# FREDZEL2020/jittor-MYC-NeRFs

Measured on AMD Instinct MI355X. Metric: ray_samples_per_sec, higher is better.
Workload: dtype f32 (emulated: 3 x f16-split MFMA products, fp32 accumulate; fp32 VALU elsewhere); 1 GPU; TensorVMSplit 300^3 (16/48 comps, MLP_Fea 150-128-128-3), 800x800 rays x 512 samples/ray (BASELINE configs[1]); ONE frame per step at every N (N>1: split over the ranks, BASELINE configs[2]), 512-ray tiles round-robin, one RCCL all_gather of [4 cap] fp32 (rgb block + depth block, written in place by the render) + two strided un-permute copies; scene=synthetic scene A (SURVEY 8d), no alpha mask, white_bg, samples_per_ray=512, rays_per_rank=640000, tile=512, chunk=640000, alpha_mask=0, emulate_world=0, arith=f32

## Files before the change

### jittor-myc-nerfs_amd/csrc/tvr_march.hip

```cpp
#include <cstdlib>
#include "tvr_device.h"
#include "tvr_kernels.h"
#include "tvr_march_body.h"
#include "tvr_gradient.h"


template <bool DENSE, bool LDSL>
__global__ __launch_bounds__(64 * MARCH_MAX_WAVES) void march_kernel(const SceneDev sc, const float *__restrict__ rays,
                                                                     const int n_rays, const int S, const int s_cap,
                                                                     const MarchSampling sm, const float eps_T,
                                                                     MarchOut mo, const tvr_dense_out dn)
{
    constexpr bool CP = false, VOL = false;
    const CpDev cp = {};
    const float *const dvol = nullptr;
#include "tvr_march_body.inc"
}

template <bool DENSE, bool PLAIN, bool BATCH>
__global__ __launch_bounds__(64 * MARCH_VOL_WAVES, DENSE ? MARCH_VOL_OCC - 1 : MARCH_VOL_OCC) void march_vol_kernel(const SceneDev sc, const float *__restrict__ dvol, const float *__restrict__ rays,
                                                                         const int n_rays, const int S, const int s_cap, const MarchSampling sm, const float eps_T,
                                                                         MarchOut mo, const tvr_dense_out dn)
{
    static_assert(!(PLAIN && DENSE), "the plain form has no dense outputs");
    constexpr bool LDSL = false, CP = false, VOL = true, MARCH_BATCH = BATCH;
    const CpDev cp = {};
#include "tvr_march_body.inc"
}

__global__ __launch_bounds__(256) void density_volume_kernel(const SceneDev sc, float *__restrict__ out)
{
    const long long gx1 = sc.grid[0] + 1, gy1 = sc.grid[1] + 1, gz1 = sc.grid[2] + 1;
    const long long t = (long long)blockIdx.x * blockDim.x + threadIdx.x;
    if (t >= gx1 * gy1 * gz1) return;
    const long long x = t % gx1, y = (t / gx1) % gy1, z = t / (gx1 * gy1);
    const float4 *P[3] = {sc.dplane[0] + (y * gx1 + x) * 4, sc.dplane[1] + (z * gx1 + x) * 4, sc.dplane[2] + (z * gy1 + y) * 4};
    const float4 *Ln[3] = {sc.dline[0] + z * 4, sc.dline[1] + y * 4, sc.dline[2] + x * 4};
    double acc = 0.0;
#pragma unroll
    for (int i = 0; i < 3; ++i) {
#pragma unroll
        for (int g = 0; g < 4; ++g) {
            const float4 p = P[i][g], l = Ln[i][g];
            acc = acc + (double)p.x * (double)l.x;
            acc = acc + (double)p.y * (double)l.y;
            acc = acc + (double)p.z * (double)l.z;
            acc = acc + (double)p.w * (double)l.w;
        }
    }
    out[t] = (float)acc;
}

hipError_t launch_density_volume(const SceneDev &sc, float *out, hipStream_t stream)
{
    const long long n = ((long long)sc.grid[0] + 1) * ((long long)sc.grid[1] + 1) * ((long long)sc.grid[2] + 1);
    hipLaunchKernelGGL(density_volume_kernel, dim3((unsigned)((n + 255) / 256)), dim3(256), 0, stream, sc, out);
    return hipGetLastError();
}

#define COMP_LANES 8
__global__ __launch_bounds__(256) void composite_kernel(const MarchOut mo, const int n_rays, const int white_bg,
                                                        float *__restrict__ rgb_out)
{
    const int t = blockIdx.x * blockDim.x + threadIdx.x;
    const int r = t / COMP_LANES, l = t % COMP_LANES;
    const bool live = r < n_rays;
    const unsigned base = live ? mo.ray_off[r] : 0u, cnt = live ? mo.ray_cnt[r] : 0u;
    float c0 = 0.f, c1 = 0.f, c2 = 0.f;
    unsigned i = l;
    for (; i + 3 * COMP_LANES < cnt; i += 4 * COMP_LANES) {
        const float4 e0 = mo.q_out[base + i], e1 = mo.q_out[base + i + COMP_LANES], e2 = mo.q_out[base + i + 2 * COMP_LANES],
                     e3 = mo.q_out[base + i + 3 * COMP_LANES];
        c0 = c0 + e0.w * e0.x; c1 = c1 + e0.w * e0.y; c2 = c2 + e0.w * e0.z;
        c0 = c0 + e1.w * e1.x; c1 = c1 + e1.w * e1.y; c2 = c2 + e1.w * e1.z;
        c0 = c0 + e2.w * e2.x; c1 = c1 + e2.w * e2.y; c2 = c2 + e2.w * e2.z;
        c0 = c0 + e3.w * e3.x; c1 = c1 + e3.w * e3.y; c2 = c2 + e3.w * e3.z;
    }
    for (; i < cnt; i += COMP_LANES) {
        const float4 e = mo.q_out[base + i];
        c0 = c0 + e.w * e.x;
        c1 = c1 + e.w * e.y;
        c2 = c2 + e.w * e.z;
    }
#pragma unroll
    for (int off = 1; off < COMP_LANES; off <<= 1) {
        c0 = c0 + __shfl_xor(c0, off);
        c1 = c1 + __shfl_xor(c1, off);
        c2 = c2 + __shfl_xor(c2, off);
    }
    if (!live || l != 0) return;
    if (mo.counter[2] != 0u) {
        const float qnan = __int_as_float(0x7fc00000);
        rgb_out[(size_t)r * 3 + 0] = qnan; rgb_out[(size_t)r * 3 + 1] = qnan; rgb_out[(size_t)r * 3 + 2] = qnan;
        mo.depth[r] = qnan;
        return;
    }
    const float acc = mo.acc[r];
    if (white_bg) {
        const float bg = 1.0f - acc;
        c0 = c0 + bg; c1 = c1 + bg; c2 = c2 + bg;
    }
    rgb_out[(size_t)r * 3 + 0] = clamp01(c0);
    rgb_out[(size_t)r * 3 + 1] = clamp01(c1);
    rgb_out[(size_t)r * 3 + 2] = clamp01(c2);
}

__global__ __launch_bounds__(256) void scatter_rgb_kernel(const MarchOut mo, const int S, float *__restrict__ rgb_dense)
{
    const unsigned n = *mo.counter;
    for (unsigned e = blockIdx.x * blockDim.x + threadIdx.x; e < n; e += gridDim.x * blockDim.x) {
        const float4 v = mo.q_out[e];
        const size_t q = ((size_t)mo.q_ray[e] * S + mo.q_j[e]) * 3;
        rgb_dense[q] = v.x; rgb_dense[q + 1] = v.y; rgb_dense[q + 2] = v.z;
    }
}

__global__ __launch_bounds__(256) void density_feature_kernel(const SceneDev sc, const float *__restrict__ xyz, const long long m,
                                                              float *__restrict__ out)
{
    const long long t = (long long)blockIdx.x * blockDim.x + threadIdx.x;
    const long long s = t >> 2;
    const int sub = threadIdx.x & 3;
    float part = 0.0f;
    if (s < m) {
        int i0[3];
        float w[3];
#pragma unroll
        for (int k = 0; k < 3; ++k) {
            const float f = unnorm(xyz[s * 3 + k], sc.gm1[k]);
            const float fl = floorf(fminf(fmaxf(f, -2.0f), sc.gm1[k] + 2.0f));
            i0[k] = (int)fl;
            w[k] = f - fl;
        }
        const float4 a = vm_term<4, true>(sc.dplane[0], sc.dline[0], sc.grid[0], sc.grid[1], sc.grid[2], i0[0], i0[1], i0[2], w[0], w[1], w[2], sub);
        const float4 b = vm_term<4, true>(sc.dplane[1], sc.dline[1], sc.grid[0], sc.grid[2], sc.grid[1], i0[0], i0[2], i0[1], w[0], w[2], w[1], sub);
        const float4 c = vm_term<4, true>(sc.dplane[2], sc.dline[2], sc.grid[1], sc.grid[2], sc.grid[0], i0[1], i0[2], i0[0], w[1], w[2], w[0], sub);
        part = ((a.x + a.y) + (a.z + a.w)) + ((b.x + b.y) + (b.z + b.w)) + ((c.x + c.y) + (c.z + c.w));
    }
    part += __shfl_xor(part, 1);
    part += __shfl_xor(part, 2);
    if (s < m && sub == 0) out[s] = part;
}

__global__ __launch_bounds__(256) void density_gradient_kernel(const SceneDev sc, const float *__restrict__ xyz, const long long m, const float3 h, const float3 inv2h,
                                                               float *__restrict__ sigma_feature, float *__restrict__ grad)
{
    const long long t = (long long)blockIdx.x * blockDim.x + threadIdx.x;
    const long long s = t >> 2;
    const int sub = threadIdx.x & 3;
    float f[7];
#pragma unroll
    for (int j = 0; j < 7; ++j) f[j] = 0.0f;
    if (s < m) vm_grad_point(sc, xyz[s * 3], xyz[s * 3 + 1], xyz[s * 3 + 2], h, sub, f);
#pragma unroll
    for (int j = 0; j < 7; ++j) {
        f[j] += __shfl_xor(f[j], 1);
        f[j] += __shfl_xor(f[j], 2);
    }
    if (s < m && sub == 0) {
        if (sigma_feature) sigma_feature[s] = f[0];
        grad[s * 3 + 0] = (f[1] - f[2]) * inv2h.x;
        grad[s * 3 + 1] = (f[3] - f[4]) * inv2h.y;
        grad[s * 3 + 2] = (f[5] - f[6]) * inv2h.z;
    }
}

__global__ __launch_bounds__(256) void alpha_sample_kernel(const SceneDev sc, const float *__restrict__ xyz, const long long m,
                                                           float *__restrict__ out)
{
    const long long s = (long long)blockIdx.x * blockDim.x + threadIdx.x;
    if (s >= m) return;
    const float p[3] = {xyz[s * 3], xyz[s * 3 + 1], xyz[s * 3 + 2]};
    out[s] = alpha_lookup(sc, p);
}

__global__ __launch_bounds__(256) void alpha_bits_kernel(const float *__restrict__ vol, const long long n, unsigned *__restrict__ bits)
{
    const long long wd = (long long)blockIdx.x * blockDim.x + threadIdx.x;
    if (wd * 32 >= n) return;
    unsigned v = 0u;
    for (int b = 0; b < 32; ++b) {
        const long long i = wd * 32 + b;
        if (i < n && vol[i] > 0.0f) v |= 1u << b;
    }
    bits[wd] = v;
}

hipError_t launch_alpha_bits(const float *vol, long long n, unsigned *bits, hipStream_t stream)
{
    const long long words = (n + 31) / 32;
    hipLaunchKernelGGL(alpha_bits_kernel, dim3((unsigned)((words + 255) / 256)), dim3(256), 0, stream, vol, n, bits);
    return hipGetLastError();
}

template <bool DENSE, bool LDSL>
static hipError_t launch_march_t(const SceneDev &sc, const float *rays, int n_rays, int S, const MarchSampling &sm, float eps_T, const MarchOut &mo,
                                 const tvr_dense_out &dn, int waves, size_t lds, unsigned grid, hipStream_t stream)
{
    hipError_t rc = hipFuncSetAttribute((const void *)march_kernel<DENSE, LDSL>, hipFuncAttributeMaxDynamicSharedMemorySize, (int)lds);
    if (rc != hipSuccess) return rc;
    hipLaunchKernelGGL((march_kernel<DENSE, LDSL>), dim3(grid), dim3(64 * waves), lds, stream, sc, rays, n_rays, S, S, sm, eps_T, mo, dn);
    return hipGetLastError();
}

static int device_cu_count()
{
    static int cus = 0;
    if (cus == 0) {
        int dev = 0, n = 0;
        if (hipGetDevice(&dev) == hipSuccess && hipDeviceGetAttribute(&n, hipDeviceAttributeMultiprocessorCount, dev) == hipSuccess && n > 0) cus = n;
        else cus = 256;
    }
    return cus;
}

int march_cu_count() { return device_cu_count(); }

static hipError_t launch_march_vol(const SceneDev &sc, const float *dvol, const float *rays, int n_rays, int S, const MarchSampling &sm, float eps_T, const MarchOut &mo,
                                   const tvr_dense_out *dense, hipStream_t stream)
{
    const int groups = MARCH_VOL_GROUPS;
    const size_t kLds = 160 * 1024 / (size_t)groups, per_list = (size_t)S * 6, fixed = MARCH_HDR + 64;
    const int n_tiles = (n_rays + MARCH_TILE - 1) / MARCH_TILE;
    int waves = 1;
    size_t lds = 0;
    long long grid = 1;
    auto shape = [&](size_t per_pend) {
        const int w = (int)((kLds - fixed - (per_pend ? 16 : 0)) / (per_list + per_pend));
        waves = w >= MARCH_VOL_WAVES ? MARCH_VOL_WAVES : (w >= 8 ? 8 : (w >= 4 ? 4 : (w >= 2 ? 2 : 1)));
        lds = per_pend ? fixed + (((size_t)waves * per_list + 15) & ~(size_t)15) + (size_t)waves * per_pend : fixed + (size_t)waves * per_list;
        grid = (long long)device_cu_count() * groups * (MARCH_VOL_WAVES / waves);
        if (grid > n_tiles) grid = n_tiles;
        if (grid < 1) grid = 1;
    };
    shape(0);
    const bool batch = (long long)n_rays > grid * (long long)waves;
    if (batch) shape((size_t)MARCH_PEND * MARCH_PEND_WORDS * 4);
    tvr_dense_out none = {};
    const tvr_dense_out &dn = dense ? *dense : none;
    const unsigned long long vol_bytes = 4ull * (unsigned long long)(sc.grid[0] + 1) * (unsigned long long)(sc.grid[1] + 1) * (unsigned long long)(sc.grid[2] + 1);
    const bool plain = !dense && sc.avol == nullptr && sm.zv == nullptr && mo.lam6 == nullptr && vol_bytes < (1ull << 32);
    hipError_t rc = hipSuccess;
    auto go = [&](auto kern) {
        rc = hipFuncSetAttribute((const void *)kern, hipFuncAttributeMaxDynamicSharedMemorySize, (int)lds);
        if (rc == hipSuccess) hipLaunchKernelGGL(kern, dim3((unsigned)grid), dim3(64 * waves), lds, stream, sc, dvol, rays, n_rays, S, S, sm, eps_T, mo, dn);
    };
    if (dense) batch ? go(march_vol_kernel<true, false, true>) : go(march_vol_kernel<true, false, false>);
    else if (plain) batch ? go(march_vol_kernel<false, true, true>) : go(march_vol_kernel<false, true, false>);
    else batch ? go(march_vol_kernel<false, false, true>) : go(march_vol_kernel<false, false, false>);
    if (rc != hipSuccess) return rc;
    return hipGetLastError();
}

hipError_t launch_march(const SceneDev &sc, const float *rays, int n_rays, int S, const MarchSampling &sm, float eps_T,
                        const MarchOut &mo, const tvr_dense_out *dense, hipStream_t stream, const float *dvol)
{
    if (dvol) return launch_march_vol(sc, dvol, rays, n_rays, S, sm, eps_T, mo, dense, stream);
    const size_t kLds = 160 * 1024, line_bytes = ((size_t)sc.grid[0] + sc.grid[1] + sc.grid[2] + 3) * 16 * MARCH_LSTRIDE, per_wave = (size_t)S * 6;
    bool ldsl = MARCH_HDR + line_bytes + 4 * per_wave + 64 <= kLds;
    const size_t fixed = MARCH_HDR + (ldsl ? line_bytes : 0) + 64;
    int waves = (int)((kLds - fixed) / per_wave);
    waves = waves >= 16 ? 16 : (waves >= 12 ? 12 : (waves >= 8 ? 8 : (waves >= 4 ? 4 : (waves >= 2 ? 2 : 1))));
    const size_t lds = fixed + (size_t)waves * per_wave;
    const int n_tiles = (n_rays + MARCH_TILE - 1) / MARCH_TILE;
    long long grid = (long long)device_cu_count() * (16 / waves > 0 ? 16 / waves : 1);
    if (grid > n_tiles) grid = n_tiles;
    if (grid < 1) grid = 1;
    tvr_dense_out none = {};
    const tvr_dense_out &dn = dense ? *dense : none;
    if (dense) return ldsl ? launch_march_t<true, true>(sc, rays, n_rays, S, sm, eps_T, mo, dn, waves, lds, (unsigned)grid, stream)
                           : launch_march_t<true, false>(sc, rays, n_rays, S, sm, eps_T, mo, dn, waves, lds, (unsigned)grid, stream);
    return ldsl ? launch_march_t<false, true>(sc, rays, n_rays, S, sm, eps_T, mo, dn, waves, lds, (unsigned)grid, stream)
                : launch_march_t<false, false>(sc, rays, n_rays, S, sm, eps_T, mo, dn, waves, lds, (unsigned)grid, stream);
}

hipError_t launch_composite(const MarchOut &mo, int n_rays, int white_bg, float *rgb, hipStream_t stream)
{
    const long long threads = (long long)n_rays * COMP_LANES;
    hipLaunchKernelGGL(composite_kernel, dim3((unsigned)((threads + 255) / 256)), dim3(256), 0, stream, mo, n_rays, white_bg, rgb);
    return hipGetLastError();
}

hipError_t launch_scatter_rgb(const MarchOut &mo, int S, float *rgb_dense, hipStream_t stream)
{
    hipLaunchKernelGGL(scatter_rgb_kernel, dim3(1024), dim3(256), 0, stream, mo, S, rgb_dense);
    return hipGetLastError();
}

hipError_t launch_density_feature(const SceneDev &sc, const float *xyz, long long m, float *out, hipStream_t stream)
{
    const long long blocks = (m * 4 + 255) / 256;
    hipLaunchKernelGGL(density_feature_kernel, dim3((unsigned)blocks), dim3(256), 0, stream, sc, xyz, m, out);
    return hipGetLastError();
}

hipError_t launch_density_gradient(const SceneDev &sc, const float *xyz, long long m, const float h[3], const float inv2h[3], float *sigma_feature, float *grad,
                                   hipStream_t stream)
{
    const long long blocks = (m * 4 + 255) / 256;
    hipLaunchKernelGGL(density_gradient_kernel, dim3((unsigned)blocks), dim3(256), 0, stream, sc, xyz, m, make_float3(h[0], h[1], h[2]),
                       make_float3(inv2h[0], inv2h[1], inv2h[2]), sigma_feature, grad);
    return hipGetLastError();
}

hipError_t launch_alpha_sample(const SceneDev &sc, const float *xyz, long long m, float *out, hipStream_t stream)
{
    hipLaunchKernelGGL(alpha_sample_kernel, dim3((unsigned)((m + 255) / 256)), dim3(256), 0, stream, sc, xyz, m, out);
    return hipGetLastError();
}
```

### jittor-myc-nerfs_amd/csrc/tvr_march_body.h

```cpp
#pragma once
#include "tvr_device.h"
#include "tvr_kernels.h"

#define MARCH_MAX_WAVES 16
#define MARCH_TILE 16
#define MARCH_SPIN_LIMIT (1u << 22)
#define MARCH_SLOTS 64u
#ifndef MARCH_CTR_WORD
#define MARCH_CTR_WORD 1
#endif
#ifndef MARCH_TAIL
#define MARCH_TAIL 4u
#endif
#ifndef MARCH_VOL_WAVES
#define MARCH_VOL_WAVES 16
#endif
#ifndef MARCH_VOL_GROUPS
#define MARCH_VOL_GROUPS 1
#endif
#ifndef MARCH_VOL_OCC
#define MARCH_VOL_OCC 8
#endif
#define MARCH_HDR 560
#ifndef MARCH_LSTRIDE
#define MARCH_LSTRIDE 4
#endif

__device__ __forceinline__ float4 vm_term_lds(const float4 *__restrict__ P, const float4 *Ls, int W, int x0, int y0, int l0,
                                              float wx, float wy, float wl, int sub)
{
    const float ux = 1.0f - wx, uy = 1.0f - wy, ul = 1.0f - wl;
    const int Wp = W + 1;
    const unsigned cell = __umul24((unsigned)y0, (unsigned)Wp) + (unsigned)x0;
    unsigned o0 = (cell << 6) + ((unsigned)sub << 4), o1 = o0 + ((unsigned)Wp << 6);
    asm volatile("" : "+v"(o0), "+v"(o1));
    const unsigned char *pb = (const unsigned char *)P;
    const float4 t00 = *(const float4 *)(pb + (size_t)o0), t01 = *(const float4 *)(pb + (size_t)o0 + 64);
    const float4 t10 = *(const float4 *)(pb + (size_t)o1), t11 = *(const float4 *)(pb + (size_t)o1 + 64);
    const float4 *q = Ls + l0 * MARCH_LSTRIDE + sub;
    const float4 l0v = q[0], l1v = q[MARCH_LSTRIDE];
    float4 p4 = f4_mul(ux * uy, t00);
    p4 = f4_fma(wx * uy, t01, p4);
    p4 = f4_fma(ux * wy, t10, p4);
    p4 = f4_fma(wx * wy, t11, p4);
    float4 q4 = f4_mul(ul, l0v);
    q4 = f4_fma(wl, l1v, q4);
    return make_float4(p4.x * q4.x, p4.y * q4.y, p4.z * q4.z, p4.w * q4.w);
}

__device__ __forceinline__ float cp_density_quad(const SceneDev &sc, const CpDev &cp, int ix, int iy, int iz, float wx, float wy, float wz, int sub)
{
    const int tpt = cp.rd >> 2;
    const float4 *__restrict__ l0 = sc.dline[0] + (size_t)iz * tpt + sub;
    const float4 *__restrict__ l1 = sc.dline[1] + (size_t)iy * tpt + sub;
    const float4 *__restrict__ l2 = sc.dline[2] + (size_t)ix * tpt + sub;
    const float ux = 1.0f - wx, uy = 1.0f - wy, uz = 1.0f - wz;
    float part = 0.0f;
    for (int g = 0; g < tpt; g += 4) {
        const float4 a0 = l0[g], a1 = l0[g + tpt], b0 = l1[g], b1 = l1[g + tpt], c0 = l2[g], c1 = l2[g + tpt];
        const float4 a = f4_fma(wz, a1, f4_mul(uz, a0)), b = f4_fma(wy, b1, f4_mul(uy, b0)), c = f4_fma(wx, c1, f4_mul(ux, c0));
        const float tx = (a.x * b.x) * c.x, ty = (a.y * b.y) * c.y, tz = (a.z * b.z) * c.z, tw = (a.w * b.w) * c.w;
        part = part + ((tx + ty) + (tz + tw));
    }
    return part;
}

struct __attribute__((packed, aligned(4))) vol_pair { float a, b; };
__device__ __forceinline__ float vol_density(const float *__restrict__ D, int gx1, int gy1, int ix, int iy, int iz, float wx, float wy, float wz)
{
    const size_t sy = (size_t)gx1, sz = (size_t)gx1 * (size_t)gy1;
    const float *r = D + ((size_t)iz * sz + (size_t)iy * sy + (size_t)ix);
    const vol_pair p00 = *(const vol_pair *)r, p01 = *(const vol_pair *)(r + sy);
    const vol_pair p10 = *(const vol_pair *)(r + sz), p11 = *(const vol_pair *)(r + sz + sy);
    const float c00 = __builtin_fmaf(wx, p00.b - p00.a, p00.a), c01 = __builtin_fmaf(wx, p01.b - p01.a, p01.a);
    const float c10 = __builtin_fmaf(wx, p10.b - p10.a, p10.a), c11 = __builtin_fmaf(wx, p11.b - p11.a, p11.a);
    const float c0 = __builtin_fmaf(wy, c01 - c00, c00), c1 = __builtin_fmaf(wy, c11 - c10, c10);
    return __builtin_fmaf(wz, c1 - c0, c0);
}

constexpr bool PLAIN = false;

constexpr bool MARCH_BATCH = false;
#define MARCH_PEND 8
#define MARCH_PEND_WORDS 12

struct MarchVolArgs {
    SceneDev sc;
    const float *dvol, *rays;
    int n_rays, S, s_cap;
    MarchSampling sm;
    float eps_T;
    MarchOut mo;
    tvr_dense_out dn;
};
template <bool ON_DEMAND, typename T>
__device__ __forceinline__ T march_arg_now(const T &arg, unsigned offset)
{
#if defined(__HIP_DEVICE_COMPILE__)
    if constexpr (ON_DEMAND) {
        const __attribute__((address_space(4))) unsigned char *ka = (const __attribute__((address_space(4))) unsigned char *)__builtin_amdgcn_kernarg_segment_ptr();
        asm volatile("" : "+s"(ka));
        return *(const __attribute__((address_space(4))) T *)(ka + offset);
    }
#endif
    return arg;
}

__device__ __forceinline__ float vol_density32(const unsigned char *r00, const unsigned char *r01, const unsigned char *r10, const unsigned char *r11, unsigned gx1,
                                               unsigned gy1, int ix, int iy, int iz, float wx, float wy, float wz)
{
    const unsigned row = __umul24((unsigned)iz, gy1) + (unsigned)iy;
    unsigned o = (row * gx1 + (unsigned)ix) << 2;
    asm volatile("" : "+v"(o));
    const vol_pair p00 = *(const vol_pair *)(r00 + (size_t)o), p01 = *(const vol_pair *)(r01 + (size_t)o);
    const vol_pair p10 = *(const vol_pair *)(r10 + (size_t)o), p11 = *(const vol_pair *)(r11 + (size_t)o);
    const float c00 = __builtin_fmaf(wx, p00.b - p00.a, p00.a), c01 = __builtin_fmaf(wx, p01.b - p01.a, p01.a);
    const float c10 = __builtin_fmaf(wx, p10.b - p10.a, p10.a), c11 = __builtin_fmaf(wx, p11.b - p11.a, p11.a);
    const float c0 = __builtin_fmaf(wy, c01 - c00, c00), c1 = __builtin_fmaf(wy, c11 - c10, c10);
    return __builtin_fmaf(wz, c1 - c0, c0);
}

#ifndef MARCH_VOL_LEAN
#define MARCH_VOL_LEAN 1
#endif
__device__ __forceinline__ float march_expf(float x)
{
    const float p = x * 0x1.715476p+0f;
    const float r = __builtin_rintf(p);
    float lo = __builtin_fmaf(x, 0x1.715476p+0f, -p);
    lo = __builtin_fmaf(x, 0x1.4ae0bep-26f, lo);
    return __builtin_ldexpf(__builtin_amdgcn_exp2f((p - r) + lo), (int)r);
}
__device__ __forceinline__ float march_softplus(float x)
{
    if (x > 20.0f) return x;
    const float t = march_expf(x);
    const float u = 1.0f + t, d = u - 1.0f;
    const float rc = __builtin_amdgcn_rcpf(d);
    float q = t * rc;
    q = __builtin_fmaf(__builtin_fmaf(-d, q, t), rc, q);
    const float lg = __builtin_amdgcn_logf(u) * 0x1.62e430p-1f;
    return d == 0.0f ? t : lg * q;
}

#define MARCH_DPP_WAVE_SHR1 0x138
#define MARCH_DPP_SAME 0xE4
template <int CTRL, int ROWS>
__device__ __forceinline__ float march_dpp_mov(float old, float v)
{
    return __int_as_float(__builtin_amdgcn_update_dpp(__float_as_int(old), __float_as_int(v), CTRL, ROWS, 0xF, false));
}
template <int N>
__device__ __forceinline__ float march_up(float v)
{
    float t = march_dpp_mov<MARCH_DPP_WAVE_SHR1, 0xF>(1.0f, v);
#pragma unroll
    for (int i = 1; i < N; ++i) t = march_dpp_mov<MARCH_DPP_WAVE_SHR1, 0xF>(t, t);
    return t;
}
__device__ __forceinline__ void scan_mul_dpp(float &x, float &excl, float &last)
{
    x = x * march_up<1>(x);
    x = x * march_up<2>(x);
    x = x * march_up<4>(x);
    x = x * march_up<8>(x);
    {
        const auto q = __builtin_amdgcn_permlane16_swap(__float_as_uint(x), __float_as_uint(x), false, false);
        const auto s = __builtin_amdgcn_permlane32_swap(q[0], q[1], false, false);
        float t = march_dpp_mov<MARCH_DPP_SAME, 0x6>(1.0f, __uint_as_float(s[0]));
        t = march_dpp_mov<MARCH_DPP_SAME, 0x8>(t, __uint_as_float(q[0]));
        x = x * t;
    }
    {
        const auto h = __builtin_amdgcn_permlane32_swap(__float_as_uint(x), __float_as_uint(x), false, false);
        x = x * march_dpp_mov<MARCH_DPP_SAME, 0xC>(1.0f, __uint_as_float(h[0]));
    }
    excl = march_up<1>(x);
    last = __int_as_float(__builtin_amdgcn_readlane(__float_as_int(x), 63));
}

template <bool PLAIN_F>
__device__ __forceinline__ void march_flush(const SceneDev &sc, const MarchSampling &sm, const MarchOut &mo, const int S, const int s_cap, const int lane, const float *bufw,
                                            const unsigned short *bufj, const float *pend, int &ring_head, int &pend_total, int &n_pend)
{
    __builtin_amdgcn_fence(__ATOMIC_ACQ_REL, "wavefront");
    const MarchOut mf = march_arg_now<PLAIN_F>(mo, offsetof(MarchVolArgs, mo));
    const bool jit_f = march_arg_now<PLAIN_F>(sm.jitter, offsetof(MarchVolArgs, sm.jitter)) != nullptr;
    const int f_total = __builtin_amdgcn_readfirstlane(pend_total), f_rays = __builtin_amdgcn_readfirstlane(n_pend), f_head = __builtin_amdgcn_readfirstlane(ring_head);
    unsigned fbase = 0;
    if (lane == 0) fbase = atomicAdd(mf.counter, (unsigned)f_total);
    fbase = __builtin_amdgcn_readfirstlane(fbase);
    if (lane < f_rays) mf.ray_off[__float_as_uint(pend[lane * MARCH_PEND_WORDS + 8])] = fbase + __float_as_uint(pend[lane * MARCH_PEND_WORDS + 9]);
    for (int i = lane; i < f_total; i += 64) {
        int k = 0;
        for (int m = 1; m < f_rays; ++m) k += (unsigned)i >= __float_as_uint(pend[m * MARCH_PEND_WORDS + 9]) ? 1 : 0;
        const float *rec = pend + k * MARCH_PEND_WORDS;
        int rp = f_head + i;
        if (rp >= s_cap) rp -= s_cap;
        const unsigned ej = bufj[rp];
        const unsigned eray = __float_as_uint(rec[8]);
        float fj = (float)ej;
        if (jit_f) fj = fj + rec[7];
        const float *__restrict__ zr = (!PLAIN_F && sm.zv) ? sm.zv + (size_t)eray * S : nullptr;
        const float z = zr ? zr[ej] : rec[6] + sc.step * fj;
        float4 qv;
        qv.x = ((rec[0] + rec[3] * z) - sc.lo[0]) * sc.inv[0] - 1.0f;
        qv.y = ((rec[1] + rec[4] * z) - sc.lo[1]) * sc.inv[1] - 1.0f;
        qv.z = ((rec[2] + rec[5] * z) - sc.lo[2]) * sc.inv[2] - 1.0f;
        qv.w = bufw[rp];
        mf.q_pos[fbase + i] = qv;
        mf.q_ray[fbase + i] = eray;
        if (mf.q_j) mf.q_j[fbase + i] = ej;
    }
    __builtin_amdgcn_fence(__ATOMIC_ACQ_REL, "wavefront");
    ring_head = f_head + f_total >= s_cap ? f_head + f_total - s_cap : f_head + f_total;
    pend_total = 0;
    n_pend = 0;
    asm volatile("" : "+v"(ring_head), "+v"(pend_total), "+v"(n_pend));
}
```

### jittor-myc-nerfs_amd/csrc/tvr_march_body.inc

```
    static_assert(!(CP && LDSL), "the CP lines (up to 96 channels) do not go through LDS");
    static_assert(!(VOL && (CP || LDSL)), "the baked volume replaces the factored evaluation: no lines in LDS, no CP lines");
    extern __shared__ __attribute__((aligned(16))) unsigned char lds_raw[];
    const int lane = threadIdx.x & 63;
    const int wave = __builtin_amdgcn_readfirstlane(threadIdx.x >> 6);
    const int n_waves = blockDim.x >> 6;
    unsigned *cursor = (unsigned *)lds_raw;
    const float4 *ls0 = (const float4 *)(lds_raw + MARCH_HDR);
    const int ln0 = LDSL ? (sc.grid[2] + 1) * MARCH_LSTRIDE : 0, ln1 = LDSL ? (sc.grid[1] + 1) * MARCH_LSTRIDE : 0, ln2 = LDSL ? (sc.grid[0] + 1) * MARCH_LSTRIDE : 0;
    const float4 *ls1 = ls0 + ln0, *ls2 = ls1 + ln1;
    float *bufw = (float *)(ls2 + ln2) + (size_t)wave * s_cap;
    unsigned short *bufj = (unsigned short *)((float *)(ls2 + ln2) + (size_t)n_waves * s_cap) + (size_t)wave * s_cap;
#ifdef TVR_MARCH_TIMELINE
    unsigned long long tl_chunks = 0ull, tl_rays = 0ull, tl_resv = 0ull;
    if (mo.stats && threadIdx.x == 0) mo.stats[32 + 8 * blockIdx.x] = __builtin_amdgcn_s_memrealtime();
#endif
    if (threadIdx.x == 0) *cursor = 0u;
    unsigned long long *slots = (unsigned long long *)(lds_raw + 16);
    if (threadIdx.x < MARCH_SLOTS) slots[threadIdx.x] = 0ull;
    unsigned long long *gstat = (unsigned long long *)(lds_raw + 16 + 8 * MARCH_SLOTS);
    if (threadIdx.x < 3) gstat[threadIdx.x] = 0ull;
    if (LDSL) {
        float4 *dst = (float4 *)(lds_raw + MARCH_HDR);
        for (int i = threadIdx.x; i < (sc.grid[2] + 1) * 4; i += blockDim.x) dst[(i >> 2) * MARCH_LSTRIDE + (i & 3)] = sc.dline[0][i];
        for (int i = threadIdx.x; i < (sc.grid[1] + 1) * 4; i += blockDim.x) dst[ln0 + (i >> 2) * MARCH_LSTRIDE + (i & 3)] = sc.dline[1][i];
        for (int i = threadIdx.x; i < (sc.grid[0] + 1) * 4; i += blockDim.x) dst[ln0 + ln1 + (i >> 2) * MARCH_LSTRIDE + (i & 3)] = sc.dline[2][i];
    }
    __syncthreads();
#ifdef TVR_MARCH_TIMELINE
    if (mo.stats && threadIdx.x == 0) mo.stats[32 + 8 * blockIdx.x + 1] = __builtin_amdgcn_s_memrealtime();
#endif
    const int sub = lane & 3;
    const unsigned char *vrow[4] = {nullptr, nullptr, nullptr, nullptr};
    if constexpr (PLAIN) {
        const size_t vsy = (size_t)(sc.grid[0] + 1) * 4, vsz = vsy * (size_t)(sc.grid[1] + 1);
        vrow[0] = (const unsigned char *)dvol; vrow[1] = vrow[0] + vsy; vrow[2] = vrow[0] + vsz; vrow[3] = vrow[2] + vsy;
    }
    unsigned long long clk0 = 0ull, ref0 = 0ull;
    if (march_arg_now<PLAIN>(mo.stats, offsetof(MarchVolArgs, mo.stats)) && threadIdx.x == 0) { clk0 = __builtin_amdgcn_s_memtime(); ref0 = __builtin_amdgcn_s_memrealtime(); }

    unsigned long long st_eval = 0, st_bbox = 0, st_term = 0;
    int last_start = 0;

    int ring_head = 0, pend_total = 0, n_pend = 0;
    float *pend = nullptr;
    if constexpr (MARCH_BATCH) {
        pend = (float *)(lds_raw + ((MARCH_HDR + (size_t)n_waves * s_cap * 6 + 15) & ~(size_t)15)) + (size_t)wave * (MARCH_PEND * MARCH_PEND_WORDS);
        asm volatile("" : "+v"(ring_head), "+v"(pend_total), "+v"(n_pend));
    }

    for (;;) {
        unsigned ci = 0;
        if (lane == 0) ci = atomicAdd(cursor, 1u);
        ci = __builtin_amdgcn_readfirstlane(ci);
        int ray_start, ray_len;
        {
            const unsigned k = ci / MARCH_TILE, slot = k & (MARCH_SLOTS - 1u);
            if ((ci % MARCH_TILE) == 0u) {
                unsigned t = 0, len = MARCH_TILE;
                if (lane == 0) {
                    if ((long long)n_rays >= 8LL * MARCH_TILE * (long long)gridDim.x && (long long)last_start + 2LL * MARCH_TILE * (long long)gridDim.x >= (long long)n_rays)
                        len = MARCH_TAIL;
                    t = atomicAdd(march_arg_now<PLAIN>(mo.counter, offsetof(MarchVolArgs, mo.counter)) + MARCH_CTR_WORD, len);
                    const unsigned long long genw = (unsigned long long)(k + 1u) | (len == MARCH_TAIL ? 0x80000000ull : 0ull);
#ifdef TVR_FAULT_INJECT_MARCH
                    if (blockIdx.x == 0 && k == 3u) __hip_atomic_store(&slots[slot], ((unsigned long long)(k + 1u + MARCH_SLOTS) << 32) | t, __ATOMIC_RELEASE, __HIP_MEMORY_SCOPE_WORKGROUP);
                    else
#endif
                    __hip_atomic_store(&slots[slot], (genw << 32) | t, __ATOMIC_RELEASE, __HIP_MEMORY_SCOPE_WORKGROUP);
                }
                ray_start = (int)__builtin_amdgcn_readfirstlane(t);
                ray_len = (int)__builtin_amdgcn_readfirstlane(len);
            } else {
                unsigned long long v;
                unsigned spins = 0u, fault = 0u;
                for (;;) {
                    v = __hip_atomic_load(&slots[slot], __ATOMIC_ACQUIRE, __HIP_MEMORY_SCOPE_WORKGROUP);
                    const unsigned gen = (unsigned)(v >> 32) & 0x7fffffffu;
                    if (gen == k + 1u) break;
                    if (gen > k + 1u) { fault = 1u; break; }
                    if (++spins > MARCH_SPIN_LIMIT) { fault = 2u; break; }
                    __builtin_amdgcn_s_sleep(1);
                }
                if (fault) {
                    if (lane == 0) atomicOr(march_arg_now<PLAIN>(mo.counter, offsetof(MarchVolArgs, mo.counter)) + 2, fault);
                    break;
                }
                ray_start = (int)(unsigned)v;
                ray_len = (v >> 63) ? MARCH_TAIL : MARCH_TILE;
            }
        }
        if (ray_start >= n_rays) break;
        if ((int)(ci % MARCH_TILE) >= ray_len) continue;
        last_start = ray_start;
        const int ray = ray_start + (int)(ci % MARCH_TILE);
        if (ray >= n_rays) continue;
        const float *__restrict__ const rays_r = march_arg_now<PLAIN>(rays, offsetof(MarchVolArgs, rays));
        const float *const jit_r = march_arg_now<PLAIN>(sm.jitter, offsetof(MarchVolArgs, sm.jitter));
        float o[3], d[3];
#pragma unroll
        for (int k = 0; k < 3; ++k) {
            o[k] = rays_r[(size_t)ray * 6 + k];
            d[k] = rays_r[(size_t)ray * 6 + 3 + k];
        }
        const float tmin = ray_tmin(sc, o, d);
        const bool has_jit = jit_r != nullptr;
        const float u = has_jit ? jit_r[ray] : 0.0f;
        const float *__restrict__ zrow = (!PLAIN && sm.zv) ? sm.zv + (size_t)ray * S : nullptr;
        float lam6 = 1.0f;
        int n6 = 0;

        float T = 1.0f, acc_l = 0.0f, dep_l = 0.0f;
        int napp = 0;
        bool seen = false, terminated = false;
        int c = 0;
        bool make_room = false;
        for (;;) {
        for (; c * 64 < S; ++c) {
            if constexpr (MARCH_BATCH) {
                if (__ballot(n_pend > 0 && (n_pend == MARCH_PEND || pend_total + napp + 64 > s_cap))) { make_room = true; break; }
            }
            const int j = c * 64 + lane;
            const bool inr = j < S;
            float fj = (float)j, fj1 = (float)(j + 1);
            if (has_jit) { fj = fj + u; fj1 = fj1 + u; }
            float z = tmin + sc.step * fj;
            float z1 = tmin + sc.step * fj1;
            if (zrow) {
                z = inr ? zrow[j] : 0.0f;
                z1 = (j < S - 1) ? zrow[j + 1] : z;
            }
            float p[3], n[3], f[3];
            bool bbox = inr;
#pragma unroll
            for (int k = 0; k < 3; ++k) {
                p[k] = o[k] + d[k] * z;
                bbox = bbox & !((sc.lo[k] > p[k]) | (p[k] > sc.hi[k]));
            }
            bool valid = bbox;
            if (!PLAIN && sc.avol != nullptr) {
                if (bbox) valid = sc.abits ? alpha_positive(sc, p) : (alpha_lookup(sc, p) > 0.0f);
            }
            int i0[3];
            float w[3];
#pragma unroll
            for (int k = 0; k < 3; ++k) {
                n[k] = (p[k] - sc.lo[k]) * sc.inv[k] - 1.0f;
                f[k] = unnorm(n[k], sc.gm1[k]);
                const float fl = floorf(f[k]);
                i0[k] = (int)fl;
                w[k] = f[k] - fl;
            }
            if constexpr (PLAIN) asm volatile("" : "+v"(i0[0]), "+v"(i0[1]), "+v"(i0[2]), "+v"(w[0]), "+v"(w[1]), "+v"(w[2]));
            const unsigned long long mb = __ballot(bbox), mv = __ballot(valid);
            if (DENSE) {
                const size_t q = (size_t)ray * S + j;
                if (inr) {
                    if (dn.z) dn.z[q] = z;
                    if (dn.valid) dn.valid[q] = valid;
                    if (dn.bbox_valid) dn.bbox_valid[q] = bbox;
                    if (dn.cell) { dn.cell[q * 3] = i0[0]; dn.cell[q * 3 + 1] = i0[1]; dn.cell[q * 3 + 2] = i0[2]; }
                }
            }
            st_bbox += __popcll(mb);
            if (mv == 0ull) {
                if (DENSE && inr) {
                    const size_t q = (size_t)ray * S + j;
                    if (dn.sigma_feature) dn.sigma_feature[q] = 0.f;
                    if (dn.sigma) dn.sigma[q] = 0.f;
                    if (dn.alpha) dn.alpha[q] = 0.f;
                    if (dn.weight) dn.weight[q] = 0.f;
                }
                if (mb == 0ull && seen && !DENSE) break;
                continue;
            }
            seen = true;
            st_eval += __popcll(mv);
#ifdef TVR_MARCH_TIMELINE
            tl_chunks++;
#endif

            float sf = 0.0f;
            if constexpr (VOL) {
                if constexpr (PLAIN) {
                    if (valid) sf = vol_density32(vrow[0], vrow[1], vrow[2], vrow[3], (unsigned)(sc.grid[0] + 1), (unsigned)(sc.grid[1] + 1), i0[0], i0[1], i0[2], w[0], w[1], w[2]);
                } else
                if (valid) sf = vol_density(dvol, sc.grid[0] + 1, sc.grid[1] + 1, i0[0], i0[1], i0[2], w[0], w[1], w[2]);
            } else {
#pragma unroll
                for (int k4 = 0; k4 < 4; ++k4) {
                    const bool v = quad_bcast_i((int)valid, k4) != 0;
                    if (__ballot(v) == 0ull) continue;
                    const int ix = quad_bcast_i(i0[0], k4), iy = quad_bcast_i(i0[1], k4), iz = quad_bcast_i(i0[2], k4);
                    const float wx = quad_bcast_f(w[0], k4), wy = quad_bcast_f(w[1], k4), wz = quad_bcast_f(w[2], k4);
                    float part = 0.0f;
                    if constexpr (CP) {
                        if (v) part = cp_density_quad(sc, cp, ix, iy, iz, wx, wy, wz, sub);
                    } else
                    if (v && LDSL) {
                        const float4 a = vm_term_lds(sc.dplane[0], ls0, sc.grid[0], ix, iy, iz, wx, wy, wz, sub);
                        const float4 b = vm_term_lds(sc.dplane[1], ls1, sc.grid[0], ix, iz, iy, wx, wz, wy, sub);
                        const float4 cc = vm_term_lds(sc.dplane[2], ls2, sc.grid[1], iy, iz, ix, wy, wz, wx, sub);
                        part = ((a.x + a.y) + (a.z + a.w)) + ((b.x + b.y) + (b.z + b.w)) + ((cc.x + cc.y) + (cc.z + cc.w));
                    } else if (v) {
                        const float4 a = vm_term<4, false>(sc.dplane[0], sc.dline[0], sc.grid[0], sc.grid[1], sc.grid[2], ix, iy, iz, wx, wy, wz, sub);
                        const float4 b = vm_term<4, false>(sc.dplane[1], sc.dline[1], sc.grid[0], sc.grid[2], sc.grid[1], ix, iz, iy, wx, wz, wy, sub);
                        const float4 cc = vm_term<4, false>(sc.dplane[2], sc.dline[2], sc.grid[1], sc.grid[2], sc.grid[0], iy, iz, ix, wy, wz, wx, sub);
                        part = ((a.x + a.y) + (a.z + a.w)) + ((b.x + b.y) + (b.z + b.w)) + ((cc.x + cc.y) + (cc.z + cc.w));
                    }
                    part += quad_perm_f<QUAD_XOR1>(part);
                    part += quad_perm_f<QUAD_XOR2>(part);
                    if (sub == k4) sf = part;
                }
            }

            float sigma = 0.0f;
            constexpr bool LEAN = VOL && MARCH_VOL_LEAN;
            if constexpr (LEAN) {
                if (valid) sigma = (sc.act == 0) ? march_softplus(sf + sc.shift) : fmaxf(sf, 0.0f);
            } else
            if (valid) sigma = (sc.act == 0) ? softplus_f(sf + sc.shift) : fmaxf(sf, 0.0f);
            float dist = (j < S - 1) ? (z1 - z) : 0.0f;
            dist = dist * sc.scale;
            const float alpha = 1.0f - (LEAN ? march_expf(-sigma * dist) : expf(-sigma * dist));
            const float fT = (1.0f - alpha) + 1e-10f;
            if (!PLAIN && mo.lam6) {
                float f6 = inr ? (1.0f - alpha) + 1e-6f : 1.0f;
#pragma unroll
                for (int off = 32; off > 0; off >>= 1) f6 = f6 * __shfl_xor(f6, off);
                lam6 = lam6 * f6;
                n6 += min(64, S - c * 64);
            }
            float incl = fT, excl, last;
            if constexpr (VOL) {
                scan_mul_dpp(incl, excl, last);
            } else {
#pragma unroll
                for (int off = 1; off < 64; off <<= 1) {
                    const float t = __shfl_up(incl, off);
                    if (lane >= off) incl = incl * t;
                }
                excl = __shfl_up(incl, 1);
                if (lane == 0) excl = 1.0f;
            }
            const float Tj = T * excl;
            const float wgt = alpha * Tj;
            acc_l += wgt;
            dep_l += wgt * z;
            const bool app = wgt > sc.thres;
            const unsigned long long ma = __ballot(app);
            if constexpr (MARCH_BATCH) {
                if (ma) {
                    int pos = ring_head + pend_total + napp + __popcll(ma & ((1ull << lane) - 1ull));
                    if (pos >= s_cap) pos -= s_cap;
                    if (app) { bufw[pos] = wgt; bufj[pos] = (unsigned short)j; }
                    napp += __popcll(ma);
                }
            } else
            if (ma) {
                const int pos = napp + __popcll(ma & ((1ull << lane) - 1ull));
                if (app) { bufw[pos] = wgt; bufj[pos] = (unsigned short)j; }
                napp += __popcll(ma);
            }
            if constexpr (VOL) T = T * last;
            else T = T * __shfl(incl, 63);
            if (DENSE && inr) {
                const size_t q = (size_t)ray * S + j;
                if (dn.sigma_feature) dn.sigma_feature[q] = valid ? sf : 0.f;
                if (dn.sigma) dn.sigma[q] = sigma;
                if (dn.alpha) dn.alpha[q] = alpha;
                if (dn.weight) dn.weight[q] = wgt;
            }
            if (T < eps_T) { terminated = true; ++c; break; }
        }
        if (!make_room) break;
#ifdef TVR_MARCH_TIMELINE
        tl_resv++;
#endif
        if constexpr (MARCH_BATCH) march_flush<PLAIN>(sc, sm, mo, S, s_cap, lane, bufw, bufj, pend, ring_head, pend_total, n_pend);
        make_room = false;
        }
        if (DENSE) {
            for (int cc = c; cc * 64 < S; ++cc) {
                const int j = cc * 64 + lane;
                if (j < S) {
                    const size_t q = (size_t)ray * S + j;
                    const float fjj = has_jit ? ((float)j + u) : (float)j;
                    if (dn.z) dn.z[q] = zrow ? zrow[j] : tmin + sc.step * fjj;
                    if (dn.valid) dn.valid[q] = 0;
                    if (dn.bbox_valid) dn.bbox_valid[q] = 0;
                    if (dn.cell) { dn.cell[q * 3] = 0; dn.cell[q * 3 + 1] = 0; dn.cell[q * 3 + 2] = 0; }
                    if (dn.sigma_feature) dn.sigma_feature[q] = 0.f;
                    if (dn.sigma) dn.sigma[q] = 0.f;
                    if (dn.alpha) dn.alpha[q] = 0.f;
                    if (dn.weight) dn.weight[q] = 0.f;
                }
            }
        }
        st_term += terminated ? 1 : 0;
#ifdef TVR_MARCH_TIMELINE
        tl_rays++;
#endif

        const float acc = wave_sum(acc_l);
        const float dep = wave_sum(dep_l);
        const MarchOut mt = march_arg_now<PLAIN>(mo, offsetof(MarchVolArgs, mo));
        if constexpr (MARCH_BATCH) {
            if (lane == 0) {
                if (napp == 0) mt.ray_off[ray] = 0u;
                mt.ray_cnt[ray] = (unsigned)napp;
                mt.acc[ray] = acc;
                mt.depth[ray] = dep + (1.0f - acc) * d[2];
                if (!PLAIN && mt.lam6) mt.lam6[ray] = lam6 * expf((float)(S - n6) * 9.5367386e-7f);
                if (DENSE) {
                    if (dn.bg_weight) dn.bg_weight[ray] = T;
                    if (dn.acc) dn.acc[ray] = acc;
                    if (dn.t_min) dn.t_min[ray] = tmin;
                }
            }
            if (napp > 0) {
                if (lane == 0) {
                    float *rec = pend + n_pend * MARCH_PEND_WORDS;
                    rec[0] = o[0]; rec[1] = o[1]; rec[2] = o[2];
                    rec[3] = d[0]; rec[4] = d[1]; rec[5] = d[2];
                    rec[6] = tmin; rec[7] = u;
                    rec[8] = __uint_as_float((unsigned)ray); rec[9] = __uint_as_float((unsigned)pend_total);
                }
                pend_total += napp;
                ++n_pend;
                asm volatile("" : "+v"(pend_total), "+v"(n_pend));
            }
            continue;
        }
        unsigned base = 0;
#ifdef TVR_MARCH_TIMELINE
        if (napp > 0) tl_resv++;
#endif
        if (lane == 0 && napp > 0) base = atomicAdd(mt.counter, (unsigned)napp);
        base = __shfl(base, 0);
        if (lane == 0) {
            mt.ray_off[ray] = base;
            mt.ray_cnt[ray] = (unsigned)napp;
            mt.acc[ray] = acc;
            mt.depth[ray] = dep + (1.0f - acc) * d[2];
            if (!PLAIN && mt.lam6) mt.lam6[ray] = lam6 * expf((float)(S - n6) * 9.5367386e-7f);
            if (DENSE) {
                if (dn.bg_weight) dn.bg_weight[ray] = T;
                if (dn.acc) dn.acc[ray] = acc;
                if (dn.t_min) dn.t_min[ray] = tmin;
            }
        }
        __builtin_amdgcn_fence(__ATOMIC_ACQ_REL, "wavefront");
        for (int i = lane; i < napp; i += 64) {
            const unsigned ej = bufj[i];
            float fj = (float)ej;
            if (has_jit) fj = fj + u;
            const float z = zrow ? zrow[ej] : tmin + sc.step * fj;
            float4 qv;
            qv.x = ((o[0] + d[0] * z) - sc.lo[0]) * sc.inv[0] - 1.0f;
            qv.y = ((o[1] + d[1] * z) - sc.lo[1]) * sc.inv[1] - 1.0f;
            qv.z = ((o[2] + d[2] * z) - sc.lo[2]) * sc.inv[2] - 1.0f;
            qv.w = bufw[i];
            mt.q_pos[base + i] = qv;
            mt.q_ray[base + i] = (unsigned)ray;
            if (mt.q_j) mt.q_j[base + i] = ej;
        }
        __builtin_amdgcn_fence(__ATOMIC_ACQ_REL, "wavefront");
    }
    if constexpr (MARCH_BATCH) {
#ifdef TVR_MARCH_TIMELINE
        if (__ballot(n_pend > 0)) tl_resv++;
#endif
        if (__ballot(n_pend > 0)) march_flush<PLAIN>(sc, sm, mo, S, s_cap, lane, bufw, bufj, pend, ring_head, pend_total, n_pend);
    }
#ifdef TVR_MARCH_TIMELINE
    if (mo.stats && lane == 0) {
        const unsigned long long te = __builtin_amdgcn_s_memrealtime();
        atomicMin((unsigned long long *)&mo.stats[32 + 8 * blockIdx.x + 2], te);
        atomicMax((unsigned long long *)&mo.stats[32 + 8 * blockIdx.x + 3], te);
        atomicAdd((unsigned long long *)&mo.stats[32 + 8 * blockIdx.x + 4], tl_chunks);
        atomicAdd((unsigned long long *)&mo.stats[32 + 8 * blockIdx.x + 5], tl_rays | (tl_resv << 32));
    }
#endif
    unsigned long long *const stats_r = march_arg_now<PLAIN>(mo.stats, offsetof(MarchVolArgs, mo.stats));
    if (stats_r) {
        if (lane == 0) {
            atomicAdd(&gstat[0], st_eval);
            atomicAdd(&gstat[1], st_bbox);
            atomicAdd(&gstat[2], st_term);
        }
        __syncthreads();
        if (threadIdx.x == 0) {
            atomicAdd((unsigned long long *)&stats_r[TVR_STAT_SAMPLES_EVAL], gstat[0]);
            atomicAdd((unsigned long long *)&stats_r[TVR_STAT_SAMPLES_BBOX], gstat[1]);
            atomicAdd((unsigned long long *)&stats_r[TVR_STAT_RAYS_TERMINATED], gstat[2]);
            atomicAdd((unsigned long long *)&stats_r[TVR_STAT_MARCH_CLK], __builtin_amdgcn_s_memtime() - clk0);
            atomicAdd((unsigned long long *)&stats_r[TVR_STAT_MARCH_REF], __builtin_amdgcn_s_memrealtime() - ref0);
        }
    }
```

Baseline: 28.60 billion ray-samples/s.

## Double the per-wave sample ring and pending queue in the batched volume march

In the batched volume-march path, the launcher now tries a per-wave LDS sample ring twice the samples-per-ray (s_cap = 2*S) with a 16-entry pending queue, as long as this does not reduce the waves per block. Otherwise it keeps the 8-entry configuration. The pending count becomes a template parameter, and the batched kernels use a different global counter word (offset 32, presumably a separate cache line). The aim is to let waves buffer more rays' samples before flushing, which smooths the MLP batch work and reduces atomic contention on the work counter. In exchange it uses more LDS and instantiates more kernel variants.

```diff
diff --git a/jittor-myc-nerfs_amd/csrc/tvr_march.hip b/jittor-myc-nerfs_amd/csrc/tvr_march.hip
--- a/jittor-myc-nerfs_amd/csrc/tvr_march.hip
+++ b/jittor-myc-nerfs_amd/csrc/tvr_march.hip
@@ -17,13 +17,15 @@
 #include "tvr_march_body.inc"
 }
 
-template <bool DENSE, bool PLAIN, bool BATCH>
+template <bool DENSE, bool PLAIN, int BATCH>
 __global__ __launch_bounds__(64 * MARCH_VOL_WAVES, DENSE ? MARCH_VOL_OCC - 1 : MARCH_VOL_OCC) void march_vol_kernel(const SceneDev sc, const float *__restrict__ dvol, const float *__restrict__ rays,
                                                                          const int n_rays, const int S, const int s_cap, const MarchSampling sm, const float eps_T,
                                                                          MarchOut mo, const tvr_dense_out dn)
 {
     static_assert(!(PLAIN && DENSE), "the plain form has no dense outputs");
-    constexpr bool LDSL = false, CP = false, VOL = true, MARCH_BATCH = BATCH;
+    constexpr bool LDSL = false, CP = false, VOL = true, MARCH_BATCH = BATCH != 0;
+    constexpr int MARCH_PEND = BATCH;
+    constexpr unsigned MARCH_CTR = BATCH ? MARCH_VOL_CTR_WORD : MARCH_CTR_WORD;
     const CpDev cp = {};
 #include "tvr_march_body.inc"
 }
@@ -225,17 +227,27 @@
     int waves = 1;
     size_t lds = 0;
     long long grid = 1;
-    auto shape = [&](size_t per_pend) {
-        const int w = (int)((kLds - fixed - (per_pend ? 16 : 0)) / (per_list + per_pend));
+    auto shape = [&](size_t per_ring, size_t per_pend) {
+        const int w = (int)((kLds - fixed - (per_pend ? 16 : 0)) / (per_ring + per_pend));
         waves = w >= MARCH_VOL_WAVES ? MARCH_VOL_WAVES : (w >= 8 ? 8 : (w >= 4 ? 4 : (w >= 2 ? 2 : 1)));
-        lds = per_pend ? fixed + (((size_t)waves * per_list + 15) & ~(size_t)15) + (size_t)waves * per_pend : fixed + (size_t)waves * per_list;
+        lds = per_pend ? fixed + (((size_t)waves * per_ring + 15) & ~(size_t)15) + (size_t)waves * per_pend : fixed + (size_t)waves * per_ring;
         grid = (long long)device_cu_count() * groups * (MARCH_VOL_WAVES / waves);
         if (grid > n_tiles) grid = n_tiles;
         if (grid < 1) grid = 1;
     };
-    shape(0);
+    shape(per_list, 0);
     const bool batch = (long long)n_rays > grid * (long long)waves;
-    if (batch) shape((size_t)MARCH_PEND * MARCH_PEND_WORDS * 4);
+    int s_cap = S, pend_n = 0;
+    if (batch) {
+        pend_n = 8;
+        shape(per_list, (size_t)pend_n * MARCH_PEND_WORDS * 4);
+        if (MARCH_VOL_RING == 2) {
+            const int waves_s = waves;
+            shape(2 * per_list, (size_t)MARCH_PEND_RING2 * MARCH_PEND_WORDS * 4);
+            if (waves == waves_s) { s_cap = 2 * S; pend_n = MARCH_PEND_RING2; }
+            else shape(per_list, (size_t)pend_n * MARCH_PEND_WORDS * 4);
+        }
+    }
     tvr_dense_out none = {};
     const tvr_dense_out &dn = dense ? *dense : none;
     const unsigned long long vol_bytes = 4ull * (unsigned long long)(sc.grid[0] + 1) * (unsigned long long)(sc.grid[1] + 1) * (unsigned long long)(sc.grid[2] + 1);
@@ -243,11 +255,12 @@
     hipError_t rc = hipSuccess;
     auto go = [&](auto kern) {
         rc = hipFuncSetAttribute((const void *)kern, hipFuncAttributeMaxDynamicSharedMemorySize, (int)lds);
-        if (rc == hipSuccess) hipLaunchKernelGGL(kern, dim3((unsigned)grid), dim3(64 * waves), lds, stream, sc, dvol, rays, n_rays, S, S, sm, eps_T, mo, dn);
+        if (rc == hipSuccess) hipLaunchKernelGGL(kern, dim3((unsigned)grid), dim3(64 * waves), lds, stream, sc, dvol, rays, n_rays, S, s_cap, sm, eps_T, mo, dn);
     };
-    if (dense) batch ? go(march_vol_kernel<true, false, true>) : go(march_vol_kernel<true, false, false>);
-    else if (plain) batch ? go(march_vol_kernel<false, true, true>) : go(march_vol_kernel<false, true, false>);
-    else batch ? go(march_vol_kernel<false, false, true>) : go(march_vol_kernel<false, false, false>);
+    auto pick = [&](auto k0, auto k8, auto k16) { pend_n == 0 ? go(k0) : (pend_n == 8 ? go(k8) : go(k16)); };
+    if (dense) pick(march_vol_kernel<true, false, 0>, march_vol_kernel<true, false, 8>, march_vol_kernel<true, false, MARCH_PEND_RING2>);
+    else if (plain) pick(march_vol_kernel<false, true, 0>, march_vol_kernel<false, true, 8>, march_vol_kernel<false, true, MARCH_PEND_RING2>);
+    else pick(march_vol_kernel<false, false, 0>, march_vol_kernel<false, false, 8>, march_vol_kernel<false, false, MARCH_PEND_RING2>);
     if (rc != hipSuccess) return rc;
     return hipGetLastError();
 }
diff --git a/jittor-myc-nerfs_amd/csrc/tvr_march_body.h b/jittor-myc-nerfs_amd/csrc/tvr_march_body.h
--- a/jittor-myc-nerfs_amd/csrc/tvr_march_body.h
+++ b/jittor-myc-nerfs_amd/csrc/tvr_march_body.h
@@ -9,6 +9,10 @@
 #ifndef MARCH_CTR_WORD
 #define MARCH_CTR_WORD 1
 #endif
+#ifndef MARCH_VOL_CTR_WORD
+#define MARCH_VOL_CTR_WORD 32
+#endif
+constexpr unsigned MARCH_CTR = MARCH_CTR_WORD;
 #ifndef MARCH_TAIL
 #define MARCH_TAIL 4u
 #endif
@@ -81,7 +85,11 @@
 constexpr bool PLAIN = false;
 
 constexpr bool MARCH_BATCH = false;
-#define MARCH_PEND 8
+constexpr int MARCH_PEND = 8;
+#define MARCH_PEND_RING2 16
+#ifndef MARCH_VOL_RING
+#define MARCH_VOL_RING 2
+#endif
 #define MARCH_PEND_WORDS 12
 
 struct MarchVolArgs {
diff --git a/jittor-myc-nerfs_amd/csrc/tvr_march_body.inc b/jittor-myc-nerfs_amd/csrc/tvr_march_body.inc
--- a/jittor-myc-nerfs_amd/csrc/tvr_march_body.inc
+++ b/jittor-myc-nerfs_amd/csrc/tvr_march_body.inc
@@ -60,7 +60,7 @@
                 if (lane == 0) {
                     if ((long long)n_rays >= 8LL * MARCH_TILE * (long long)gridDim.x && (long long)last_start + 2LL * MARCH_TILE * (long long)gridDim.x >= (long long)n_rays)
                         len = MARCH_TAIL;
-                    t = atomicAdd(march_arg_now<PLAIN>(mo.counter, offsetof(MarchVolArgs, mo.counter)) + MARCH_CTR_WORD, len);
+                    t = atomicAdd(march_arg_now<PLAIN>(mo.counter, offsetof(MarchVolArgs, mo.counter)) + MARCH_CTR, len);
                     const unsigned long long genw = (unsigned long long)(k + 1u) | (len == MARCH_TAIL ? 0x80000000ull : 0ull);
 #ifdef TVR_FAULT_INJECT_MARCH
                     if (blockIdx.x == 0 && k == 3u) __hip_atomic_store(&slots[slot], ((unsigned long long)(k + 1u + MARCH_SLOTS) << 32) | t, __ATOMIC_RELEASE, __HIP_MEMORY_SCOPE_WORKGROUP);
```

After: 28.78 billion ray-samples/s (median of 6 runs). Within noise of the previous version (+0.6%).
